# EPFL-IMOS/simple-SFOD

Hardware: AMD Instinct MI355X
Metric: teacher+student train images/s on 1024x2048 synthetic (higher is better)
Workload: dtype bf16x3

## Files before the change

### include/sfod_hip.h

```cpp
#ifndef SFOD_HIP_H
#define SFOD_HIP_H
#include <stdint.h>
#ifdef __cplusplus
extern "C" {
#endif

#define SFOD_F32 0
#define SFOD_BF16 1
#define SFOD_BF16X3 2
#define SFOD_F16X3 3

int sfod_version(void);
const char* sfod_last_error(void);

int sfod_preprocess(const void* const* img_ptrs, const int32_t* sizes, int B, int Hp, int Wp,
                    int Cpad, const float* mean3, const float* std3, void* out, int dt,
                    void* stream);

int sfod_hflip_u8(const void* src, void* dst, int C, int H, int W, void* stream);

int sfod_resize_bilinear_u8(const void* src, void* dst, int C, int H, int W, int h, int w,
                            const int32_t* hbounds, const int32_t* hcoef, int ksize_h,
                            const int32_t* vbounds, const int32_t* vcoef, int ksize_v, int flip,
                            void* stream);

int sfod_conv_fwd(const void* x, const void* w, const float* bias, void* y, int B, int H, int W,
                  int Cin, int Cout, int ksize, int ldy, int act, float* stats, int dt, int out_dt,
                  void* stream);
int sfod_conv_fwd_ws(const void* x, const void* w, const uint32_t* w_absmax, const float* bias, void* y, int B, int H,
                     int W, int Cin, int Cout, int ksize, int ldy, int act, float* stats, int dt, int out_dt,
                     void* stream);
int64_t sfod_conv_fwd_scratch_bytes(int B, int H, int W, int Cin, int Cout, int ksize, int dt, int out_dt, int with_stats);
int sfod_conv_fwd_scratch(const void* x, const void* w, const uint32_t* w_absmax, const float* bias, void* y, int B, int H,
                          int W, int Cin, int Cout, int ksize, int ldy, int act, float* stats, int dt, int out_dt,
                          void* scratch, int64_t scratch_bytes, void* stream);
int sfod_conv_stats_blocks(int B, int H, int W, int Cin, int Cout, int ksize, int dt);
int sfod_set_conv_algo(int algo);
int sfod_conv_dgrad_bnred_blocks(int B, int H, int W, int Cin, int Cout, int dt);
int sfod_conv_dgrad_bnred(const void* x, const void* w, void* dz, int B, int H, int W, int Cin, int Cout, int dt,
                          const float* y, const float* mean, const float* invstd, const float* gamma,
                          const float* beta, float* red_ws, void* stream);
int sfod_conv_fwd_bnin_supported(int B, int H, int W, int Cin, int Cout, int dt);
int sfod_conv_fwd_bnin(const float* x_pre, const float* in_mean, const float* in_invstd, const float* in_gamma,
                       const float* in_beta, const void* w, const float* bias, float* y, int B, int H, int W, int Cin,
                       int Cout, int ldy, int act, float* stats, int dt, void* stream);
int sfod_set_gemm_tile(int tile);
int sfod_set_conv3x3_variant(int variant);
int sfod_last_conv_kernel(char* buf, int n);
int sfod_set_deterministic(int on);
int sfod_get_deterministic(void);
int sfod_set_conv3x3_m16(int on);
int sfod_set_wgrad3x3_pipe(int on);
int sfod_conv_fwd_algo(int B, int H, int W, int Cin, int Cout, int ksize, int dt);

int sfod_conv_first_supported(int B, int H, int W, int Cin, int Cout, int dt, int ldy);
int sfod_conv_first_fused(const void* x, const void* w, const float* bias, const float* scale,
                          const float* shift, void* y, float* stats, int B, int H, int W, int ldy,
                          int act, int dt, void* stream);
int sfod_conv_first_fused_ws(const void* x, const void* w, const uint32_t* w_absmax, const float* bias,
                             const float* scale, const float* shift, void* y, float* stats, int B, int H, int W,
                             int ldy, int act, int dt, void* stream);

int64_t sfod_conv_wgrad_ws_bytes(int B, int H, int W, int Cin, int Cout, int ksize, int lddy, int dt);
int sfod_conv_wgrad(const void* x, const void* dy, float* dw, int B, int H, int W, int Cin,
                    int Cout, int ksize, int lddy, int dt, void* ws, int64_t ws_bytes, void* stream);
int sfod_conv_wgrad_oihw_supported(int B, int H, int W, int Cin, int Cout, int ksize, int lddy, int dt);
int sfod_conv_wgrad_oihw(const void* x, const void* dy, float* dw_oihw, int B, int H, int W, int Cin,
                         int Cout, int ksize, int lddy, int dt, int accumulate, void* ws,
// ... 173 lines not shown
```

### simple-sfod_amd/csrc/conv3x3_patch.hip

```cpp
#include "conv_internal.h"
#include <type_traits>
#include <stdlib.h>
#include <atomic>

typedef __attribute__((ext_vector_type(8))) __bf16 bf16x8;
typedef __attribute__((ext_vector_type(16))) float f32x16;
typedef __attribute__((ext_vector_type(4))) float f32x4_t;

#define LDS_PTR(p) ((__attribute__((address_space(3))) void*)(p))

namespace {

template <int J> using IC = std::integral_constant<int, J>;

constexpr int BSLOT = 8192;
constexpr int STG_PITCH = 144;

template <int G, int FM> struct Lay {
  static constexpr bool SMALL = (G == 1) ? (FM == 2) : (FM == 1);
  static constexpr int NPW = SMALL ? 3 : 5;
  static constexpr int PATCH_ROWS = NPW * 8 * 16;
  static constexpr int PATCH_BYTES = PATCH_ROWS * 64;
  static constexpr int D = SMALL ? 2 : 3;
  static constexpr int NBS = D + 1;
// ... 11 lines not shown
  const bf16_t* x;
  const bf16_t* w;
  const float* bias;
  void* y;
  float* stats;
  int B, H, W, Cin, Cout, ldy, act;
  int TH, TW, PW;
  int tiles_x, tiles_y, tiles_n;
  unsigned m_pw, m_tw, m_tn, m_tx, m_ty;
  int nbody;
  int ntiles;
  int nblk;
  const float* red_y;
  const float* red_mean;
  const float* red_invstd;
  const float* red_gamma;
  const float* red_beta;
  float* red_ws;
  const unsigned* wamax;
  const float* xf_mean;
  const float* xf_invstd;
  const float* xf_gamma;
  const float* xf_beta;
};

constexpr unsigned OOB_OFF = 0x80000000u;
__device__ __forceinline__ void bufload16(__amdgpu_buffer_rsrc_t rsrc, unsigned voff, unsigned soff, void* l) {
  __builtin_amdgcn_raw_ptr_buffer_load_lds(rsrc, LDS_PTR(l), 16, (int)voff, (int)soff, 0, 0);
}

__device__ __forceinline__ unsigned fdiv(unsigned x, unsigned d, unsigned m) { return d == 1 ? x : __umulhi(x, m); }

template <int N> __device__ __forceinline__ void wait_vm() {
  asm volatile("s_waitcnt vmcnt(%0) lgkmcnt(0)" ::"n"(N) : "memory");
}

struct ActP { float slope; bool relu; };
__device__ __forceinline__ ActP act_params(int act) { return ActP{act == 2 ? 0.2f : 1.f, act == 1}; }
__device__ __forceinline__ float act_f(float v, ActP p) { return fmaxf(v, p.relu ? 0.f : v * p.slope); }

template <int G, int FM> struct WaitTab;
template <> struct WaitTab<1, 4> {
  static constexpr int N[9] = {2, 3, 4, 4, 4, 4, 3, 2, 2};
  static constexpr int NL[9] = {2, 2, 2, 2, 2, 2, 2, 1, 0};
};
template <> struct WaitTab<2, 2> {
  static constexpr int N[9] = {1, 4, 5, 4, 1, 2, 4, 5, 4};
  static constexpr int NL[9] = {1, 4, 5, 4, 1, 2, 2, 1, 0};
};
template <> struct WaitTab<1, 2> {
  static constexpr int N[9] = {1, 2, 2, 2, 1, 1, 1, 1, 1};
  static constexpr int NL[9] = {1, 1, 1, 1, 1, 1, 1, 1, 0};
};
template <> struct WaitTab<2, 1> {
  static constexpr int N[9] = {1, 2, 2, 2, 1, 1, 2, 2, 2};
  static constexpr int NL[9] = {1, 2, 2, 2, 1, 1, 1, 1, 0};
};

template <int G, int FM, typename OutT, int SPLIT = 0, bool RED = false>
__global__ void __launch_bounds__(512, (Lay<G, FM>::SMALL ? 4 : 2))
k_conv3x3_patch(P3Args a) {
  using L = Lay<G, FM>;
  constexpr int BN = 128 / G;
  constexpr int FN = 2;
  constexpr int WROWS = FM * 32;
  constexpr int NPW = L::NPW, PATCH_BYTES = L::PATCH_BYTES, BRING_OFF = L::BRING_OFF, D = L::D, NBS = L::NBS;
  constexpr int PIXTAB_OFF = L::PIXTAB_OFF, SRED_OFF = L::SRED_OFF;
  extern __shared__ __attribute__((aligned(16))) unsigned char smem[];

  const int lane = threadIdx.x & 63;
  const int wave = __builtin_amdgcn_readfirstlane(threadIdx.x >> 6);
  const int wm = (G == 1) ? (wave >> 1) : wave;
  const int wn = (G == 1) ? (wave & 1) : 0;
  const int h = lane >> 5;

  int bid = blockIdx.x;
  {
    const int q = a.ntiles / 8, r = a.ntiles % 8, xcd = bid % 8;
    bid = (xcd < r ? xcd * (q + 1) : r * (q + 1) + (xcd - r) * q) + bid / 8;
  }
  int t = (int)fdiv((unsigned)bid, (unsigned)a.tiles_n, a.m_tn);
  const int tn = bid - t * a.tiles_n;
  int t2 = (int)fdiv((unsigned)t, (unsigned)a.tiles_x, a.m_tx);
  const int txi = t - t2 * a.tiles_x;
// ... 262 lines not shown
      }
    const bool vec_ok = (a.ldy % 8) == 0;
    bf16_t* yo = reinterpret_cast<bf16_t*>(a.y);
#pragma unroll 4
    for (int it = 0; it < WROWS / 8; ++it) {
      const int row = it * 8 + (lane >> 3), ch = lane & 7;
      const int pix = pixtab[wm * WROWS + row];
      const int n = n0 + wn * 64 + ch * 8;
      if (pix < 0 || n >= a.Cout) continue;
      const unsigned char* src = stg + row * STG_PITCH + ch * 16;
      bf16_t* dst = yo + (ybase + pix) * a.ldy + n;
      if (vec_ok && n + 8 <= a.Cout) {
        *reinterpret_cast<uint4*>(dst) = *reinterpret_cast<const uint4*>(src);
      } else {
        for (int e = 0; e < 8 && n + e < a.Cout; ++e) dst[e] = reinterpret_cast<const bf16_t*>(src)[e];
      }
    }
  } else {
    float* yo = reinterpret_cast<float*>(a.y);
    constexpr int FP = 272;
    static_assert(8 * 32 * FP <= Lay<G, FM>::STG || 8 * 32 * FP <= Lay<G, FM>::OPER, "fp32 staging must fit the operand area");
    unsigned char* stg = smem + wave * (32 * FP);
    const bool vec_ok = (a.ldy % 4) == 0;
#pragma unroll
    for (int i = 0; i < FM; ++i) {
#pragma unroll
      for (int j = 0; j < FN; ++j) {
        const int nl = j * 32 + (lane & 31);
#pragma unroll
        for (int r = 0; r < 16; ++r) {
          const int ml = (r & 3) + 8 * (r >> 2) + 4 * h;
          const float v = acc[i][j][r] + bcol[j];
          acc[i][j][r] = v;
          *reinterpret_cast<float*>(stg + ml * FP + nl * 4) = act_f(v, actp);
        }
      }
#pragma unroll
      for (int it = 0; it < 8; ++it) {
        const int row = it * 4 + (lane >> 4), ch = lane & 15;
        const int pix = pixtab[wm * WROWS + i * 32 + row];
        const int n = n0 + wn * 64 + ch * 4;
        if (pix < 0 || n >= a.Cout) continue;
        const float4 v = *reinterpret_cast<const float4*>(stg + row * FP + ch * 16);
        float* dst = yo + (ybase + pix) * a.ldy + n;
        if (vec_ok && n + 4 <= a.Cout) {
          *reinterpret_cast<float4*>(dst) = v;
        } else {
          const float e[4] = {v.x, v.y, v.z, v.w};
          for (int q = 0; q < 4 && n + q < a.Cout; ++q) dst[q] = e[q];
        }
      }
    }
  }

  if constexpr (RED) {
    static_assert(sizeof(OutT) == 4, "the reduction epilogue belongs to fp32 data-gradient launches");
    float* sred = reinterpret_cast<float*>(smem + SRED_OFF);
    const float* __restrict__ yb = a.red_y + ybase * a.ldy;
#pragma unroll
    for (int j = 0; j < FN; ++j) {
      const int n = n0 + wn * 64 + j * 32 + (lane & 31);
      const int nc = min(n, a.Cout - 1);
      const float mu = a.red_mean[nc], is = a.red_invstd[nc];
      const float sc = is * a.red_gamma[nc], sh = a.red_beta[nc];
      float sb = 0.f, sg = 0.f;
#pragma unroll
      for (int i = 0; i < FM; ++i)
#pragma unroll
        for (int r = 0; r < 16; ++r) {
          const int ml = i * 32 + (r & 3) + 8 * (r >> 2) + 4 * h;
          const int pix = pixtab[wm * WROWS + ml];
          const float yv = yb[(unsigned)(max(pix, 0) * a.ldy + nc)];
          const float d = yv - mu;
          const float g = (pix >= 0 && d * sc + sh > 0.f) ? acc[i][j][r] : 0.f;
// ... 136 lines not shown
  }
}

template <int NW, int NIP, int NWN = 2> struct M16Lay {
  static constexpr int PIX = (NW / NWN) * NIP * 16;
  static constexpr int PR = (PIX == 256) ? 384 : 640;
  static constexpr int NPW = PR / 16 / NW;
  static constexpr int PPS = (NPW + 2) / 3;
  static constexpr int PPP = 4 * NWN;
  static constexpr int WPW = 2 * PPP / NW;
  static constexpr int PATCH_BYTES = PR * 64;
  static constexpr int WR_OFF = 2 * PATCH_BYTES;
  static constexpr int WSLOT = 2 * PPP * 1024;
  static constexpr int LDS = WR_OFF + 2 * WSLOT;
  static_assert(WPW >= 1 && PPP % WPW == 0 && PPS <= 3, "a wave's weight pieces of a stage lie inside one pair");
};

#ifdef M16_STAMP
__device__ unsigned long long g_m16_stamps[8];
#endif

typedef float __attribute__((address_space(4))) cfloat_k;

template <int NW, int NIP, int FMT, bool RED, bool XF = false, int NWN = 2>
__global__ void __launch_bounds__(NW * 64, (NW * (160 * 1024 / M16Lay<NW, NIP, NWN>::LDS)) / 4 > 0 ? (NW * (160 * 1024 / M16Lay<NW, NIP, NWN>::LDS)) / 4 : 1)
k_conv3x3_m16(P3Args a) {
  using L = M16Lay<NW, NIP, NWN>;
  static_assert(!XF || NWN == 2, "the in-LDS BatchNorm transform lives in the 128-channel shape");
  static_assert(!XF || (NW == 4 && NIP == 8 && FMT == 1 && !RED), "the in-LDS BatchNorm transform lives in the 4-wave bf16-pair forward kernel");
#ifdef M16_STAMP
  const unsigned long long stamp_t0 = __builtin_amdgcn_s_memtime();
#endif
  constexpr int PR = L::PR, NPW = L::NPW, WPW = L::WPW, PATCH_BYTES = L::PATCH_BYTES, WR_OFF = L::WR_OFF, WSLOT = L::WSLOT;
  constexpr int NWM = NW / NWN;
  constexpr int PPP = L::PPP;
  constexpr int WPX = NIP * 16;
  constexpr int XB = (NIP >= 8) ? 2 : 1;
  extern __shared__ __attribute__((aligned(16))) unsigned char smem[];

  const int lane = threadIdx.x & 63;
  const int wave = __builtin_amdgcn_readfirstlane(threadIdx.x >> 6);
  const int wm = wave / NWN, wn = wave % NWN;
  const int q = lane >> 4, r16 = lane & 15;
  const int pb = q & 1, chh = q >> 1;

  int bid = blockIdx.x;
  {
    const int qq = a.ntiles / 8, r = a.ntiles % 8, xcd = bid % 8;
    bid = (xcd < r ? xcd * (qq + 1) : r * (qq + 1) + (xcd - r) * qq) + bid / 8;
  }
// ... 312 lines not shown
    }
    pix[ip] = v;
  }
  const int cb = n0 + wn * 64 + q * 4;
  float* yo = reinterpret_cast<float*>(a.y);
  const bool fast = (a.ldy % 4) == 0 && (n0 + wn * 64 + 64 <= a.Cout);
  float bv[4][4];
#pragma unroll
  for (int ic = 0; ic < 4; ++ic)
#pragma unroll
    for (int r = 0; r < 4; ++r) {
      const int c = cb + ic * 16 + r;
      bv[ic][r] = (a.bias != nullptr && c < a.Cout) ? a.bias[c] : 0.f;
    }
  int64_t rowoff[NIP];
#pragma unroll
  for (int ip = 0; ip < NIP; ++ip) rowoff[ip] = (ybase + max(pix[ip], 0)) * a.ldy;
#pragma unroll
  for (int ic = 0; ic < 4; ++ic)
#pragma unroll
    for (int ip = 0; ip < NIP; ++ip)
#pragma unroll
      for (int r = 0; r < 4; ++r) acc[ic][ip][r] += bv[ic][r];
  if (fast) {
#pragma unroll
    for (int ic = 0; ic < 4; ++ic)
#pragma unroll
      for (int ip = 0; ip < NIP; ++ip) {
        float4 o;
        o.x = act_f(acc[ic][ip][0], actp); o.y = act_f(acc[ic][ip][1], actp);
        o.z = act_f(acc[ic][ip][2], actp); o.w = act_f(acc[ic][ip][3], actp);
        if (pix[ip] >= 0) *reinterpret_cast<float4*>(yo + rowoff[ip] + (cb + ic * 16)) = o;
      }
  } else {
#pragma unroll
    for (int ic = 0; ic < 4; ++ic)
#pragma unroll
      for (int ip = 0; ip < NIP; ++ip)
#pragma unroll
        for (int r = 0; r < 4; ++r) {
          const int c = cb + ic * 16 + r;
          if (pix[ip] >= 0 && c < a.Cout) yo[rowoff[ip] + c] = act_f(acc[ic][ip][r], actp);
        }
  }

  if constexpr (!RED) { if (a.stats == nullptr) return; }
  __syncthreads();
// ... 194 lines not shown
  p.G = (variant <= 2) ? 1 : 2;
  p.FM = (variant == 1) ? 4 : (variant == 3 ? 1 : 2);
  if (Cin % (32 * p.G) != 0) return p;
  if ((int64_t)H * W * Cin >= (int64_t)1 << 30 || (int64_t)Cout * 9 * Cin >= (int64_t)1 << 30) return p;
  const int BM = (p.G == 1 ? 4 : 8) * p.FM * 32;
  const int cap = (BM == 256) ? PATCH_ROWS_SMALL : PATCH_ROWS_BIG;
  if (!p3_best_tile(H, W, BM, cap, p.TH, p.TW, p.tiles_y, p.tiles_x)) return p;
  p.tiles_n = (Cout + (128 / p.G) - 1) / (128 / p.G);
  p.nblk = B * p.tiles_y * p.tiles_x;
  p.ok = 1;
  return p;
}

#ifdef M16_STAMP
extern "C" int sfod_debug_m16_stamps(unsigned long long* out8, int reset) {
  SFOD_REQUIRE_EXTENTS("debug_m16_stamps", reset);
  hipDeviceSynchronize();
  hipMemcpyFromSymbol(out8, HIP_SYMBOL(g_m16_stamps), 64);
  if (reset) { unsigned long long z[8] = {0, 0, 0, 0, 0, 0, 0, 0}; hipMemcpyToSymbol(HIP_SYMBOL(g_m16_stamps), z, 64); }
  return 0;
}
#endif

template <int NW, int NIP, int FMT, bool RED, bool XF = false, int NWN = 2>
static int p3_launch_m16(P3Args a, hipStream_t s) {
  auto kern = k_conv3x3_m16<NW, NIP, FMT, RED, XF, NWN>;
  constexpr int LDS = M16Lay<NW, NIP, NWN>::LDS;
  static const hipError_t attr_rc =
      hipFuncSetAttribute(reinterpret_cast<const void*>(kern), hipFuncAttributeMaxDynamicSharedMemorySize, LDS);
  if (attr_rc != hipSuccess) { sfod_set_error("hipFuncSetAttribute(m16): %s", hipGetErrorString(attr_rc)); return -(int)attr_rc; }
  a.nbody = a.Cin / 64;
  static const std::string kname =
      sfod_kernel_name("k_conv3x3_m16<%d,%d,%d,%d,%d,%d>", NW, NIP, FMT, (int)RED, (int)XF, NWN);
  sfod_note_conv_kernel(kname.c_str());
  hipLaunchKernelGGL(kern, dim3(a.ntiles), dim3(NW * 64), LDS, s, a);
  return sfod_check_launch("conv3x3_m16");
}

template <int G, int FM, typename OutT, int SPLIT = 0, bool RED = false>
static int p3_launch_one(const P3Args& a, hipStream_t s) {
  auto kern = k_conv3x3_patch<G, FM, OutT, SPLIT, RED>;
  constexpr int LDS = Lay<G, FM>::TOTAL;
  static const hipError_t attr_rc =
      hipFuncSetAttribute(reinterpret_cast<const void*>(kern), hipFuncAttributeMaxDynamicSharedMemorySize, LDS);
  if (attr_rc != hipSuccess) { sfod_set_error("hipFuncSetAttribute(p3): %s", hipGetErrorString(attr_rc)); return -(int)attr_rc; }
  static const std::string kname =
      sfod_kernel_name("k_conv3x3_patch<%d,%d,%s,%d,%d>", G, FM, sfod_type_name<OutT>(), SPLIT, (int)RED);
  sfod_note_conv_kernel(kname.c_str());
  hipLaunchKernelGGL(kern, dim3(a.ntiles), dim3(512), LDS, s, a);
  return sfod_check_launch("conv3x3_patch");
}

bool sfod_p3_bnin_ok(const P3Plan& p, int Cin_phys, int split) {
  return p.ok && p.m16 != 0 && p.G == 1 && p.FM == 2 && Cin_phys % 64 == 0 && split == 1;
}

int sfod_p3_launch(const P3Plan& p, const void* x, const void* w, const float* bias, void* y, float* stats,
                   int B, int H, int W, int Cin, int Cout, int ldy, int act, int out_f32, hipStream_t s, int split,
                   const P3BnRed* red, const unsigned* wamax, const P3BnIn* bnin) {
  P3Args a;
  a.wamax = wamax;
  a.xf_mean = a.xf_invstd = a.xf_gamma = a.xf_beta = nullptr;
  if (bnin != nullptr) {
    if (!sfod_p3_bnin_ok(p, Cin, split) || red != nullptr || !out_f32) {
      sfod_set_error("conv3x3_patch: the BatchNorm-input form needs bf16x3 operands, the 256 x 128 shape, Cin % 32 == 0");
      return SFOD_EBADARG;
    }
    a.xf_mean = bnin->mean; a.xf_invstd = bnin->invstd; a.xf_gamma = bnin->gamma; a.xf_beta = bnin->beta;
  }
  a.red_y = nullptr; a.red_mean = a.red_invstd = a.red_gamma = a.red_beta = nullptr; a.red_ws = nullptr;
  if (red != nullptr) {
    if (!out_f32 || ldy != Cout || Cout % 4 != 0) { sfod_set_error("conv3x3_patch: BatchNorm-backward epilogue needs a dense fp32 output"); return SFOD_EBADARG; }
    a.red_y = red->y; a.red_mean = red->mean; a.red_invstd = red->invstd; a.red_gamma = red->gamma; a.red_beta = red->beta;
    a.red_ws = red->ws;
  }
  a.x = (const bf16_t*)x; a.w = (const bf16_t*)w; a.bias = bias; a.y = y; a.stats = stats;
  a.B = B; a.H = H; a.W = W; a.Cin = Cin; a.Cout = Cout; a.ldy = ldy; a.act = act;
  a.TH = p.TH; a.TW = p.TW; a.PW = p.TW + 2;
  a.tiles_x = p.tiles_x; a.tiles_y = p.tiles_y; a.tiles_n = p.tiles_n;
  auto magic = [](int d) { return (unsigned)((((unsigned long long)1) << 32) / (unsigned)d + 1ull); };
  a.m_pw = magic(a.PW); a.m_tw = magic(a.TW); a.m_tn = magic(a.tiles_n); a.m_tx = magic(a.tiles_x);
  a.m_ty = magic(a.tiles_y);
  a.nbody = Cin / (32 * p.G);
  a.ntiles = B * p.tiles_y * p.tiles_x * p.tiles_n;
  a.nblk = p.nblk;
  if (split) {
    if (!out_f32) { sfod_set_error("conv3x3_patch: operand pairs write fp32"); return SFOD_EBADARG; }
    if (bnin != nullptr) return p3_launch_m16<4, 8, 1, false, true>(a, s);
    if (p.m16 && p.G == 1 && p.FM == 2 && Cin % 64 == 0 && (red == nullptr || split == 1)) {
      if (p.m16 == 2) {
        if (red != nullptr) return p3_launch_m16<4, 8, 1, true>(a, s);
        return split == 2 ? p3_launch_m16<4, 8, 2, false>(a, s) : p3_launch_m16<4, 8, 1, false>(a, s);
      }
      if (red != nullptr) return p3_launch_m16<8, 4, 1, true>(a, s);
      return split == 2 ? p3_launch_m16<8, 4, 2, false>(a, s) : p3_launch_m16<8, 4, 1, false>(a, s);
    }
    if (p.m16 && p.G == 2 && Cin % 64 == 0 && (red == nullptr || split == 1) && (p.m16 >= 3 || p3_m16_n64_enabled())) {
      if (p.FM == 1 && (p.m16 == 4 || p3_m16_n64_enabled() == 2)) {
        if (red != nullptr) return p3_launch_m16<8, 2, 1, true, false, 1>(a, s);
        return split == 2 ? p3_launch_m16<8, 2, 2, false, false, 1>(a, s) : p3_launch_m16<8, 2, 1, false, false, 1>(a, s);
      }
      if (p.FM == 1) {
        if (red != nullptr) return p3_launch_m16<4, 4, 1, true, false, 1>(a, s);
        return split == 2 ? p3_launch_m16<4, 4, 2, false, false, 1>(a, s) : p3_launch_m16<4, 4, 1, false, false, 1>(a, s);
      }
      if (red != nullptr) return p3_launch_m16<8, 4, 1, true, false, 1>(a, s);
      return split == 2 ? p3_launch_m16<8, 4, 2, false, false, 1>(a, s) : p3_launch_m16<8, 4, 1, false, false, 1>(a, s);
    }
    if (red != nullptr) {
      if (split != 1) { sfod_set_error("conv3x3_patch: the BatchNorm-backward epilogue runs on bf16x3 operands"); return SFOD_EBADARG; }
      if (p.G == 1 && p.FM == 2) return p3_launch_one<1, 2, float, 1, true>(a, s);
// ... 21 lines not shown
```

### simple-sfod_amd/csrc/conv_internal.h

```cpp
#pragma once
#include "common.h"

struct P3Plan {
  int ok;
  int G;
  int FM;
  int TH, TW;
  int tiles_y, tiles_x, tiles_n;
  int nblk;
  int m16;
};
P3Plan sfod_p3_plan(int B, int H, int W, int Cin, int Cout, int pairs = 0);
struct P3BnRed {
  const float* y;
  const float* mean;
  const float* invstd;
  const float* gamma;
  const float* beta;
  float* ws;
};
struct P3BnIn {
  const float* mean;
  const float* invstd;
  const float* gamma;
  const float* beta;
};
bool sfod_p3_bnin_ok(const P3Plan& p, int Cin_phys, int split);
int sfod_p3_launch(const P3Plan& p, const void* x, const void* w, const float* bias, void* y, float* stats,
                   int B, int H, int W, int Cin, int Cout, int ldy, int act, int out_f32, hipStream_t s, int split = 0,
                   const P3BnRed* red = nullptr, const unsigned* wamax = nullptr, const P3BnIn* bnin = nullptr);


struct W3Plan {
  int ok;
  int CO;
  int TH, TW, tiles_y, tiles_x;
  int co_tiles, ci_tiles;
  int tiles_per_split, nsplit, nslab;
  int64_t ws_bytes;
  int w64;
};
W3Plan sfod_w3_plan(int B, int H, int W, int Cin, int Cout, int lddy, int split = 0);
int sfod_w3_launch(const W3Plan& p, const void* x, const void* dy, float* dw, void* ws, int B, int H, int W,
                   int Cin, int Cout, int lddy, int out_mode, hipStream_t s, int split = 0);

bool sfod_deterministic();

void sfod_f16_poll_elementwise(unsigned* out, hipStream_t s);
void sfod_f16_poll_roi(unsigned* out, hipStream_t s);
void sfod_f16_poll_first(unsigned* out, hipStream_t s);
void sfod_f16_poll_stem(unsigned* out, hipStream_t s);

int sfod_f1_nblk(int B, int H, int W);
// ... 4 lines not shown
```

### simple-sfod_amd/csrc/gemm_conv.hip

```cpp
#include "conv_internal.h"
#include <algorithm>
#include <atomic>

typedef __attribute__((ext_vector_type(8))) __bf16 bf16x8;
typedef __attribute__((ext_vector_type(4))) short s16x4;
typedef __attribute__((ext_vector_type(8))) short s16x8;
typedef __attribute__((ext_vector_type(16))) float f32x16;
typedef __attribute__((ext_vector_type(4))) float f32x4;

#define LDS_PTR(p) ((__attribute__((address_space(3))) void*)(p))
#define GLB_PTR(p) ((const __attribute__((address_space(1))) void*)(p))

__device__ __attribute__((aligned(16))) unsigned int g_zero_page[64];

struct ConvArgs {
  int M;
  int H, W;
  int Cin;
  int Cout;
  int ks;
  int cpt_shift;
  int kchunks;
  int ldy;
  int act;
// ... 732 lines not shown
extern "C" int sfod_conv_fwd_bnin_supported(int B, int H, int W, int Cin, int Cout, int dt) {
  if (!conv_shape_fits(B, H, W, Cin, Cout, 3)) return 0;
  if (dt != SFOD_BF16X3 || (int64_t)B * H * W == 0 || g_conv_algo == 1) return 0;
  const int pc = phys_ch(dt, Cin);
  const P3Plan p = sfod_p3_plan(B, H, W, pc, Cout, 1);
  return (use_patch_kernel(p, B, H, W, 3, dt) && sfod_p3_bnin_ok(p, pc, 1)) ? 1 : 0;
}

extern "C" int sfod_conv_fwd_bnin(const float* x_pre, const float* in_mean, const float* in_invstd, const float* in_gamma,
                                  const float* in_beta, const void* w, const float* bias, float* y, int B, int H, int W,
                                  int Cin, int Cout, int ldy, int act, float* stats, int dt, void* stream) {
  sfod_note_conv_kernel(nullptr);
  SFOD_REQUIRE(conv_shape_fits(B, H, W, Cin, Cout, 3) && sfod_ints_ok({ldy}), "conv_fwd_bnin: negative or oversized extent");
  SFOD_REQUIRE(sfod_conv_fwd_bnin_supported(B, H, W, Cin, Cout, dt), "conv_fwd_bnin: shape not served (sfod_conv_fwd_bnin_supported)");
  SFOD_REQUIRE(x_pre && in_mean && in_invstd && in_gamma && in_beta && w && y, "conv_fwd_bnin: null argument");
  SFOD_REQUIRE(ldy >= Cout, "conv_fwd_bnin: ldy < Cout");
  const int pc = phys_ch(dt, Cin);
  const P3Plan p = sfod_p3_plan(B, H, W, pc, Cout, 1);
  const P3BnIn bnin{in_mean, in_invstd, in_gamma, in_beta};
  return sfod_p3_launch(p, x_pre, w, bias, y, stats, B, H, W, pc, Cout, ldy, act, 1, (hipStream_t)stream, 1, nullptr, nullptr,
                        &bnin);
}

extern "C" int sfod_conv_dgrad_bnred_blocks(int B, int H, int W, int Cin, int Cout, int dt) {
  if (!conv_shape_fits(B, H, W, Cin, Cout, 3)) return 0;
  if (dt != SFOD_BF16X3 && dt != SFOD_BF16) return 0;
  if (dt == SFOD_BF16) return 0;
  if (Cout % 4 != 0) return 0;
  const P3Plan p = sfod_p3_plan(B, H, W, phys_ch(dt, Cin), Cout, sfod_is_pairs(dt));
  return use_patch_kernel(p, B, H, W, 3, dt) ? p.nblk : 0;
}

extern "C" int sfod_conv_dgrad_bnred(const void* x, const void* w, void* dz, int B, int H, int W, int Cin, int Cout,
                                     int dt, const float* y, const float* mean, const float* invstd,
                                     const float* gamma, const float* beta, float* red_ws, void* stream) {
  sfod_note_conv_kernel(nullptr);
  SFOD_REQUIRE(conv_shape_fits(B, H, W, Cin, Cout, 3), "conv_dgrad_bnred: negative or oversized extent");
  SFOD_REQUIRE(x != nullptr && w != nullptr && dz != nullptr, "conv_dgrad_bnred: null operand");
  SFOD_REQUIRE(sfod_conv_dgrad_bnred_blocks(B, H, W, Cin, Cout, dt) > 0,
               "conv_dgrad_bnred: shape not served (sfod_conv_dgrad_bnred_blocks)");
  SFOD_REQUIRE(y && mean && invstd && gamma && beta && red_ws, "conv_dgrad_bnred: null argument");
  const int pc = phys_ch(dt, Cin);
  const P3Plan p = sfod_p3_plan(B, H, W, pc, Cout, sfod_is_pairs(dt));
  const P3BnRed red{y, mean, invstd, gamma, beta, red_ws};
  return sfod_p3_launch(p, x, w, nullptr, dz, nullptr, B, H, W, pc, Cout, Cout, 0, 1, (hipStream_t)stream,
                        dt == SFOD_BF16X3, &red);
// ... 648 lines not shown
```

### simple-sfod_amd/modeling/backbone_vgg.py

```python
import os

import torch
import torch.nn as nn

from .. import native
from . import offchain as _offchain
from ..registry import BACKBONE_REGISTRY
from ..structures import ShapeSpec

VGG16 = [64, 64, "M", 128, 128, "M", 256, 256, 256, "M", 512, 512, 512, "M", 512, 512, 512, "M"]
STAGE_SLICES = [(0, 7), (7, 14), (14, 24), (24, 34), (34, 44)]


def make_layers(cfg_list, batch_norm=False):
    layers = []
    in_channels = 3
    for v in cfg_list:
        if v == "M":
            layers += [nn.MaxPool2d(kernel_size=2, stride=2)]
        else:
            conv2d = nn.Conv2d(in_channels, v, kernel_size=3, padding=1)
            if batch_norm:
                layers += [conv2d, nn.BatchNorm2d(v), nn.ReLU(inplace=True)]
            else:
# ... 44 lines not shown
        self._initialize_weights()
        chans, strides = [64, 128, 256, 512, 512], [2, 4, 8, 16, 32]
        mods = list(self.vgg._modules.values())
        self.stages = [nn.Sequential(*mods[a:b]) for a, b in STAGE_SLICES]
        self._out_feature_channels, self._out_feature_strides, self._stage_names = {}, {}, []
        for i, stage in enumerate(self.stages):
            name = "vgg{}".format(i)
            self.add_module(name, stage)
            self._stage_names.append(name)
            self._out_feature_channels[name] = chans[i]
            self._out_feature_strides[name] = strides[i]
        self._out_features = self._stage_names
        self.needed_features = set(self._stage_names)
        del self.vgg
        self.compute_dtype = native.mode_dtype(cfg.SFOD.COMPUTE_DTYPE)
        self.grad_dtype = native.grad_dtype_of(self.compute_dtype)
        self.bn_momentum, self.bn_eps = 0.1, 1e-5
        self.bn_updates_per_forward = 1
        self.fuse_first = bool(cfg.SFOD.FUSE_FIRST_LAYER) if "SFOD" in cfg and "FUSE_FIRST_LAYER" in cfg.SFOD else True
        self.fuse_bn_input = bool(cfg.SFOD.FUSE_BN_INPUT) if "SFOD" in cfg and "FUSE_BN_INPUT" in cfg.SFOD else True
        self.fuse_bn_input_min_bytes = int(os.environ.get("SFOD_BNIN_MIN_BYTES", str(256 << 20)))
        self.wgrad_stream = os.environ.get("SFOD_VGG_WGRAD_STREAM", "1") != "0"
        self.fuse_bn_reduce = os.environ.get("SFOD_NO_FUSE_BN_REDUCE", "0") != "1"
        self._plan = []
        for s, stage in enumerate(self.stages):
            ms = list(stage)
            i = 0
            while i < len(ms):
                if isinstance(ms[i], nn.Conv2d):
                    pool = i + 3 < len(ms) and isinstance(ms[i + 3], nn.MaxPool2d)
                    self._plan.append([ms[i], ms[i + 1], pool, False])
                    i += 4 if pool else 3
                else:
                    i += 1
            self._plan[-1][3] = True

    @property
    def size_divisibility(self):
        return 0

    def output_shape(self):
        return {n: ShapeSpec(channels=self._out_feature_channels[n], stride=self._out_feature_strides[n])
                for n in self._out_features}

    def _initialize_weights(self):
        for m in self.modules():
# ... 58 lines not shown
            fwd = [(conv.weight, cin0_pad if li == 0 else conv.in_channels, False)
                   for li, (conv, _, _, _) in enumerate(self._plan)]
            rot = [(conv.weight, conv.out_channels, True) for conv, _, _, _ in self._plan[1:]] if with_dgrad else []
            if gdt == dt or not rot:
                pk = (native.ConvWeightPacker(fwd + rot, dt), None)
            else:
                pk = (native.ConvWeightPacker(fwd, dt), native.ConvWeightPacker(rot, gdt))
            packers[key] = pk
        views = list(pk[0].pack()) + (list(pk[1].pack()) if pk[1] is not None else [])
        n = len(self._plan)
        return views[:n], ([None] + list(views[n:]) if with_dgrad else None)

    def _defer_bn(self, li, y, fwd_w, save, training):
        if save or not training or not self.fuse_bn_input or li + 1 >= len(self._plan):
            return False
        _, _, pool, stage_end = self._plan[li]
        if pool or stage_end:
            return False
        if y.numel() * 4 < self.fuse_bn_input_min_bytes:
            return False
        nxt = self._plan[li + 1][0]
        return native.conv_fwd_bnin_supported(y, fwd_w[li + 1], nxt.out_channels)

    def _forward_impl(self, x, save=True):
        dt = native.dt_of(x)
        training = self.training
        saved, outs = [], []
        fwd_w, rot_w = self._packed_weights(dt, x.shape[-1], save)
        self._rot_w = rot_w
        x_g = native.as_operand(x, self.grad_dtype) if save else None
        pending = None
        for li, (conv, bn, pool, stage_end) in enumerate(self._plan):
            cout = conv.out_channels
            wp = fwd_w[li]
            if pending is not None:
                yb, mb, ib, bnb = pending
                pending = None
                B, H, W, _ = yb.shape
                y, stats = native.conv_fwd_bnin(yb, mb, ib, bnb.weight.detach(), bnb.bias.detach(), wp, conv.bias.detach(),
                                                cout, want_stats=True)
                mean, invstd = native.bn_finalize(stats, B * H * W, cout, bn.running_mean, bn.running_var,
                                                  self.bn_momentum, self.bn_eps, self.bn_updates_per_forward,
                                                  num_batches_tracked=bn.num_batches_tracked)
                if self._defer_bn(li, y, fwd_w, save, training):
                    pending = (y, mean, invstd, bn)
                    continue
                x = native.bn_relu_pool_fwd(y, mean, invstd, bn.weight.detach(), bn.bias.detach(), pool, out_dtype=x.dtype)
                if stage_end:
                    outs.append(x)
                continue
            B, H, W, _ = x.shape
            if (li == 0 and training and not save and not pool and not stage_end and self.fuse_first
                    and native.conv_first_supported(x, cout)):
                stats = native.conv_first_stats(x, wp, conv.bias.detach())
                mean, invstd = native.bn_finalize(stats, B * H * W, cout, bn.running_mean, bn.running_var,
                                                  self.bn_momentum, self.bn_eps, self.bn_updates_per_forward,
                                                  num_batches_tracked=bn.num_batches_tracked)
                scale = bn.weight.detach() * invstd
                shift = bn.bias.detach() - mean * scale
                x = native.conv_first_apply(x, wp, conv.bias.detach(), scale, shift, relu=True)
                continue
            if training:
                y, stats = native.conv_fwd(x, wp, conv.bias.detach(), cout, 3, want_stats=True)
                mean, invstd = native.bn_finalize(stats, B * H * W, cout, bn.running_mean, bn.running_var,
                                                  self.bn_momentum, self.bn_eps, self.bn_updates_per_forward,
                                                  num_batches_tracked=bn.num_batches_tracked)
            else:
                y = native.conv_fwd(x, wp, conv.bias.detach(), cout, 3)
                mean = bn.running_mean
                invstd = torch.rsqrt(bn.running_var + self.bn_eps)
            if self._defer_bn(li, y, fwd_w, save, training):
                pending = (y, mean, invstd, bn)
                continue
            zz = native.bn_relu_pool_fwd(y, mean, invstd, bn.weight.detach(), bn.bias.detach(), pool,
# ... 96 lines not shown
```

### simple-sfod_amd/native.py

```python
import ctypes
import os
import re
import warnings

import torch

warnings.filterwarnings("ignore", message="ComplexHalf support is experimental")

_HERE = os.path.dirname(os.path.abspath(__file__))
HEADER = os.path.join(os.path.dirname(_HERE), "include", "sfod_hip.h")
SO_PATH = os.environ.get("SFOD_HIP_LIB", os.path.join(_HERE, "lib", "libsfod_hip.so"))

F32, BF16, BF16X3, F16X3 = 0, 1, 2, 3

SPLIT_DTYPE = torch.complex32
SPLITH_DTYPE = torch.uint32
PAIR_DTYPES = (SPLIT_DTYPE, SPLITH_DTYPE)

COMPUTE_MODES = {"fp32": F32, "bf16": BF16, "bf16x3": BF16X3, "f16x3": F16X3}


def mode_dt(name):
    try:
        return COMPUTE_MODES[str(name).lower()]
# ... 538 lines not shown
    _pending_flops = 2.0 * B * H * W * cout * ksize * ksize * cin
    if _timer is not None:
        _pending_tag = ":patch3x3" if query("sfod_conv_fwd_algo", B, H, W, cin, cout, ksize, dt) == 2 else ":gemm"
    odt = dt_of_dtype(out_dtype)
    nscratch = load().sfod_conv_fwd_scratch_bytes(B, H, W, cin, cout, ksize, dt, odt, int(want_stats)) if ksize == 1 else 0
    if nscratch > 0:
        scratch = torch.empty(nscratch, dtype=torch.uint8, device=x.device)
        call("sfod_conv_fwd_scratch", x, w_packed, wscale_of(w_packed), bias, y, B, H, W, cin, cout, ksize, ldy, act, stats,
             dt, odt, scratch, nscratch, timer_name="sfod_conv_fwd")
    else:
        call("sfod_conv_fwd_ws", x, w_packed, wscale_of(w_packed), bias, y, B, H, W, cin, cout, ksize, ldy, act, stats, dt,
             odt, timer_name="sfod_conv_fwd")
    _pending_tag = ""
    return (y, stats) if want_stats else y


def conv_fwd_bnin_supported(y_pre, w_packed, cout):
    if y_pre.dim() != 4 or y_pre.dtype != torch.float32 or w_packed.dtype != SPLIT_DTYPE:
        return False
    B, H, W, cin = y_pre.shape
    return bool(query("sfod_conv_fwd_bnin_supported", B, H, W, cin, cout, BF16X3))


def conv_fwd_bnin(y_pre, mean, invstd, gamma, beta, w_packed, bias, cout, act=0, want_stats=False):
    B, H, W, cin = y_pre.shape
    y = torch.empty((B, H, W, cout), dtype=torch.float32, device=y_pre.device)
    stats = None
    if want_stats:
        nb = query("sfod_conv_stats_blocks", B, H, W, cin, cout, 3, BF16X3)
        stats = torch.empty(nb * (2 * cout + 1), dtype=torch.float32, device=y_pre.device)
        stats.nblk = nb
    global _pending_flops, _pending_tag
    _pending_flops = 2.0 * B * H * W * cout * 9 * cin
    _pending_tag = ":patch3x3"
    try:
        call("sfod_conv_fwd_bnin", y_pre, mean, invstd, gamma, beta, w_packed, bias, y, B, H, W, cin, cout, cout, act, stats,
             BF16X3, timer_name="sfod_conv_fwd")
    finally:
        _pending_tag = ""
    return (y, stats) if want_stats else y


def conv_first_supported(x, cout):
    if x.dim() != 4 or x.dtype not in (torch.bfloat16,) + PAIR_DTYPES:
        return False
    B, H, W, cin = x.shape
    return bool(query("sfod_conv_first_supported", B, H, W, cin, cout, dt_of(x), cout))


def conv_first_stats(x, w_packed, bias):
    B, H, W, cin = x.shape
    nb = query("sfod_conv_stats_blocks", B, H, W, cin, 64, 3, dt_of(x))
    stats = torch.empty(nb * (2 * 64 + 1), dtype=torch.float32, device=x.device)
    stats.nblk = nb
    call("sfod_conv_first_fused_ws", x, w_packed, wscale_of(w_packed), bias, None, None, None, stats, B, H, W, 64, 0,
         dt_of(x))
    return stats


def conv_first_apply(x, w_packed, bias, scale, shift, relu=True):
    B, H, W, cin = x.shape
    z = torch.empty(B, H, W, 64, dtype=x.dtype, device=x.device)
    global _pending_flops
# ... 536 lines not shown
```

Before: 160.4.

## Fuse 2x2 max-pool into conv3x3 forward epilogue for teacher forward

Adds a pooling epilogue to the patch and m16 3x3 conv kernels. Each 2x2 window is reduced with a sign-aware max, using the BN gamma sign so the max commutes with the later affine BN, and only the pooled map is written. The backbone uses it when no activations are saved (the teacher forward), so the full-resolution fp32 conv output is never written or reread by the pool pass. The cost is extra epilogue work, LDS staging or DPP shuffles, and new template instantiations. Correctness depends on the sign trick and on BN statistics still being gathered at full resolution.

Measured after the change: 161.6, median of 6. About the same (+0.8%).

```diff
diff --git a/include/sfod_hip.h b/include/sfod_hip.h
--- a/include/sfod_hip.h
+++ b/include/sfod_hip.h
@@ -44,6 +44,12 @@
 int sfod_conv_fwd_bnin(const float* x_pre, const float* in_mean, const float* in_invstd, const float* in_gamma,
                        const float* in_beta, const void* w, const float* bias, float* y, int B, int H, int W, int Cin,
                        int Cout, int ldy, int act, float* stats, int dt, void* stream);
+int sfod_conv_fwd_pool_supported(int B, int H, int W, int Cin, int Cout, int dt, int bnin);
+int sfod_conv_fwd_pool(const void* x, const void* w, const float* bias, const float* pool_gamma, float* y_pooled, int B,
+                       int H, int W, int Cin, int Cout, int ldy, float* stats, int dt, void* stream);
+int sfod_conv_fwd_bnin_pool(const float* x_pre, const float* in_mean, const float* in_invstd, const float* in_gamma,
+                            const float* in_beta, const void* w, const float* bias, const float* pool_gamma, float* y_pooled,
+                            int B, int H, int W, int Cin, int Cout, int ldy, float* stats, int dt, void* stream);
 int sfod_set_gemm_tile(int tile);
 int sfod_set_conv3x3_variant(int variant);
 int sfod_last_conv_kernel(char* buf, int n);
diff --git a/simple-sfod_amd/csrc/conv3x3_patch.hip b/simple-sfod_amd/csrc/conv3x3_patch.hip
--- a/simple-sfod_amd/csrc/conv3x3_patch.hip
+++ b/simple-sfod_amd/csrc/conv3x3_patch.hip
@@ -57,7 +57,15 @@
   const float* xf_invstd;
   const float* xf_gamma;
   const float* xf_beta;
+  const float* pool_gamma;
 };
+
+__device__ __forceinline__ unsigned pool_sign(const float* g, int n, int Cout) {
+  return (n < Cout) ? (__builtin_bit_cast(unsigned, g[n]) & 0x80000000u) : 0u;
+}
+__device__ __forceinline__ float pool_flip(float v, unsigned sg) {
+  return __builtin_bit_cast(float, __builtin_bit_cast(unsigned, v) ^ sg);
+}
 
 constexpr unsigned OOB_OFF = 0x80000000u;
 __device__ __forceinline__ void bufload16(__amdgpu_buffer_rsrc_t rsrc, unsigned voff, unsigned soff, void* l) {
@@ -92,9 +100,10 @@
   static constexpr int NL[9] = {1, 2, 2, 2, 1, 1, 1, 1, 0};
 };
 
-template <int G, int FM, typename OutT, int SPLIT = 0, bool RED = false>
+template <int G, int FM, typename OutT, int SPLIT = 0, bool RED = false, bool POOL = false>
 __global__ void __launch_bounds__(512, (Lay<G, FM>::SMALL ? 4 : 2))
 k_conv3x3_patch(P3Args a) {
+  static_assert(!POOL || (G == 2 && FM == 1 && sizeof(OutT) == 4 && !RED), "the pooling epilogue lives in the 256 x 64 fp32 forward shape");
   using L = Lay<G, FM>;
   constexpr int BN = 128 / G;
   constexpr int FN = 2;
@@ -403,6 +412,49 @@
     static_assert(8 * 32 * FP <= Lay<G, FM>::STG || 8 * 32 * FP <= Lay<G, FM>::OPER, "fp32 staging must fit the operand area");
     unsigned char* stg = smem + wave * (32 * FP);
     const bool vec_ok = (a.ldy % 4) == 0;
+    if constexpr (POOL) {
+#pragma unroll
+      for (int j = 0; j < FN; ++j) {
+        const int nl = j * 32 + (lane & 31);
+#pragma unroll
+        for (int r = 0; r < 16; ++r) {
+          const int ml = (r & 3) + 8 * (r >> 2) + 4 * h;
+          const float v = acc[0][j][r] + bcol[j];
+          acc[0][j][r] = v;
+          *reinterpret_cast<float*>(stg + ml * FP + nl * 4) = v;
+        }
+      }
+      __syncthreads();
+      const int pw2 = a.TW >> 1, np2 = (a.TH >> 1) * pw2;
+      const int Hp = a.H >> 1, Wp = a.W >> 1;
+      for (int it = threadIdx.x; it < np2 * 16; it += 512) {
+        const int pp = it >> 4, ch = it & 15;
+        const int pr = pp / pw2, pc = pp - pr * pw2;
+        const int ty = 2 * pr, tx = 2 * pc;
+        const int n = n0 + ch * 4;
+        if (y0 + ty + 1 >= a.H || x0 + tx + 1 >= a.W || n >= a.Cout) continue;
+        const unsigned char* src = smem + (ty * a.TW + tx) * FP + ch * 16;
+        const float4 v00 = *reinterpret_cast<const float4*>(src), v01 = *reinterpret_cast<const float4*>(src + FP);
+        const float4 v10 = *reinterpret_cast<const float4*>(src + a.TW * FP);
+        const float4 v11 = *reinterpret_cast<const float4*>(src + (a.TW + 1) * FP);
+        const float e00[4] = {v00.x, v00.y, v00.z, v00.w}, e01[4] = {v01.x, v01.y, v01.z, v01.w};
+        const float e10[4] = {v10.x, v10.y, v10.z, v10.w}, e11[4] = {v11.x, v11.y, v11.z, v11.w};
+        float o[4];
+#pragma unroll
+        for (int q = 0; q < 4; ++q) {
+          const unsigned sg = pool_sign(a.pool_gamma, n + q, a.Cout);
+          const float m = fmaxf(fmaxf(pool_flip(e00[q], sg), pool_flip(e01[q], sg)),
+                                fmaxf(pool_flip(e10[q], sg), pool_flip(e11[q], sg)));
+          o[q] = pool_flip(m, sg);
+        }
+        float* dst = yo + (((int64_t)b * Hp + ((y0 + ty) >> 1)) * Wp + ((x0 + tx) >> 1)) * a.ldy + n;
+        if (vec_ok && n + 4 <= a.Cout) {
+          *reinterpret_cast<float4*>(dst) = make_float4(o[0], o[1], o[2], o[3]);
+        } else {
+          for (int q = 0; q < 4 && n + q < a.Cout; ++q) dst[q] = o[q];
+        }
+      }
+    } else {
 #pragma unroll
     for (int i = 0; i < FM; ++i) {
 #pragma unroll
@@ -431,6 +483,7 @@
           for (int q = 0; q < 4 && n + q < a.Cout; ++q) dst[q] = e[q];
         }
       }
+    }
     }
   }
 
@@ -613,10 +666,11 @@
 
 typedef float __attribute__((address_space(4))) cfloat_k;
 
-template <int NW, int NIP, int FMT, bool RED, bool XF = false, int NWN = 2>
+template <int NW, int NIP, int FMT, bool RED, bool XF = false, int NWN = 2, bool POOL = false>
 __global__ void __launch_bounds__(NW * 64, (NW * (160 * 1024 / M16Lay<NW, NIP, NWN>::LDS)) / 4 > 0 ? (NW * (160 * 1024 / M16Lay<NW, NIP, NWN>::LDS)) / 4 : 1)
 k_conv3x3_m16(P3Args a) {
   using L = M16Lay<NW, NIP, NWN>;
+  static_assert(!POOL || (NW == 4 && NIP == 8 && NWN == 2 && !RED), "the pooling epilogue lives in the 4-wave 256 x 128 forward shape");
   static_assert(!XF || NWN == 2, "the in-LDS BatchNorm transform lives in the 128-channel shape");
   static_assert(!XF || (NW == 4 && NIP == 8 && FMT == 1 && !RED), "the in-LDS BatchNorm transform lives in the 4-wave bf16-pair forward kernel");
 #ifdef M16_STAMP
@@ -975,7 +1029,41 @@
     for (int ip = 0; ip < NIP; ++ip)
 #pragma unroll
       for (int r = 0; r < 4; ++r) acc[ic][ip][r] += bv[ic][r];
-  if (fast) {
+  if constexpr (POOL) {
+    const int Hp = a.H >> 1, Wp = a.W >> 1;
+    unsigned sg[4][4];
+#pragma unroll
+    for (int ic = 0; ic < 4; ++ic)
+#pragma unroll
+      for (int r = 0; r < 4; ++r) sg[ic][r] = pool_sign(a.pool_gamma, cb + ic * 16 + r, a.Cout);
+#pragma unroll
+    for (int ipp = 0; ipp < NIP / 2; ++ipp) {
+      const int ip = (ipp >> 1) * 4 + (ipp & 1);
+      const int p = wm * WPX + ip * 16 + r16;
+      const int ty = p >> 5, tx = p & 31;
+      const bool ok = (r16 & 1) == 0 && ty + 1 < a.TH && y0 + ty + 1 < a.H && x0 + tx + 1 < a.W;
+      const int64_t off = (((int64_t)b * Hp + ((y0 + ty) >> 1)) * Wp + ((x0 + tx) >> 1)) * a.ldy;
+#pragma unroll
+      for (int ic = 0; ic < 4; ++ic) {
+        float o[4];
+#pragma unroll
+        for (int r = 0; r < 4; ++r) {
+          float m = fmaxf(pool_flip(acc[ic][ip][r], sg[ic][r]), pool_flip(acc[ic][ip + 2][r], sg[ic][r]));
+          m = fmaxf(m, __builtin_bit_cast(float, __builtin_amdgcn_update_dpp(0, __builtin_bit_cast(int, m), 0xB1, 0xF, 0xF, true)));
+          o[r] = pool_flip(m, sg[ic][r]);
+        }
+        if (ok) {
+          if (fast) {
+            *reinterpret_cast<float4*>(yo + off + (cb + ic * 16)) = make_float4(o[0], o[1], o[2], o[3]);
+          } else {
+#pragma unroll
+            for (int r = 0; r < 4; ++r)
+              if (cb + ic * 16 + r < a.Cout) yo[off + cb + ic * 16 + r] = o[r];
+          }
+        }
+      }
+    }
+  } else if (fast) {
 #pragma unroll
     for (int ic = 0; ic < 4; ++ic)
 #pragma unroll
@@ -1216,30 +1304,32 @@
 }
 #endif
 
-template <int NW, int NIP, int FMT, bool RED, bool XF = false, int NWN = 2>
+template <int NW, int NIP, int FMT, bool RED, bool XF = false, int NWN = 2, bool POOL = false>
 static int p3_launch_m16(P3Args a, hipStream_t s) {
-  auto kern = k_conv3x3_m16<NW, NIP, FMT, RED, XF, NWN>;
+  auto kern = k_conv3x3_m16<NW, NIP, FMT, RED, XF, NWN, POOL>;
   constexpr int LDS = M16Lay<NW, NIP, NWN>::LDS;
   static const hipError_t attr_rc =
       hipFuncSetAttribute(reinterpret_cast<const void*>(kern), hipFuncAttributeMaxDynamicSharedMemorySize, LDS);
   if (attr_rc != hipSuccess) { sfod_set_error("hipFuncSetAttribute(m16): %s", hipGetErrorString(attr_rc)); return -(int)attr_rc; }
   a.nbody = a.Cin / 64;
-  static const std::string kname =
-      sfod_kernel_name("k_conv3x3_m16<%d,%d,%d,%d,%d,%d>", NW, NIP, FMT, (int)RED, (int)XF, NWN);
+  static const std::string kname = POOL
+      ? sfod_kernel_name("k_conv3x3_m16<%d,%d,%d,%d,%d,%d,1>", NW, NIP, FMT, (int)RED, (int)XF, NWN)
+      : sfod_kernel_name("k_conv3x3_m16<%d,%d,%d,%d,%d,%d>", NW, NIP, FMT, (int)RED, (int)XF, NWN);
   sfod_note_conv_kernel(kname.c_str());
   hipLaunchKernelGGL(kern, dim3(a.ntiles), dim3(NW * 64), LDS, s, a);
   return sfod_check_launch("conv3x3_m16");
 }
 
-template <int G, int FM, typename OutT, int SPLIT = 0, bool RED = false>
+template <int G, int FM, typename OutT, int SPLIT = 0, bool RED = false, bool POOL = false>
 static int p3_launch_one(const P3Args& a, hipStream_t s) {
-  auto kern = k_conv3x3_patch<G, FM, OutT, SPLIT, RED>;
+  auto kern = k_conv3x3_patch<G, FM, OutT, SPLIT, RED, POOL>;
   constexpr int LDS = Lay<G, FM>::TOTAL;
   static const hipError_t attr_rc =
       hipFuncSetAttribute(reinterpret_cast<const void*>(kern), hipFuncAttributeMaxDynamicSharedMemorySize, LDS);
   if (attr_rc != hipSuccess) { sfod_set_error("hipFuncSetAttribute(p3): %s", hipGetErrorString(attr_rc)); return -(int)attr_rc; }
-  static const std::string kname =
-      sfod_kernel_name("k_conv3x3_patch<%d,%d,%s,%d,%d>", G, FM, sfod_type_name<OutT>(), SPLIT, (int)RED);
+  static const std::string kname = POOL
+      ? sfod_kernel_name("k_conv3x3_patch<%d,%d,%s,%d,%d,1>", G, FM, sfod_type_name<OutT>(), SPLIT, (int)RED)
+      : sfod_kernel_name("k_conv3x3_patch<%d,%d,%s,%d,%d>", G, FM, sfod_type_name<OutT>(), SPLIT, (int)RED);
   sfod_note_conv_kernel(kname.c_str());
   hipLaunchKernelGGL(kern, dim3(a.ntiles), dim3(512), LDS, s, a);
   return sfod_check_launch("conv3x3_patch");
@@ -1249,11 +1339,25 @@
   return p.ok && p.m16 != 0 && p.G == 1 && p.FM == 2 && Cin_phys % 64 == 0 && split == 1;
 }
 
+bool sfod_p3_pool_ok(const P3Plan& p, int Cin_phys, int split, bool bnin) {
+  if (!p.ok || split != 1 || (p.TH & 1) || (p.TW & 1)) return false;
+  if (bnin) return sfod_p3_bnin_ok(p, Cin_phys, split) && p.TW == 32;
+  if (p.G != 2 || p.FM != 1 || Cin_phys % 64 != 0) return false;
+  return !(p.m16 && (p.m16 >= 3 || p3_m16_n64_enabled()));
+}
+
 int sfod_p3_launch(const P3Plan& p, const void* x, const void* w, const float* bias, void* y, float* stats,
                    int B, int H, int W, int Cin, int Cout, int ldy, int act, int out_f32, hipStream_t s, int split,
-                   const P3BnRed* red, const unsigned* wamax, const P3BnIn* bnin) {
+                   const P3BnRed* red, const unsigned* wamax, const P3BnIn* bnin, const float* pool_gamma) {
   P3Args a;
   a.wamax = wamax;
+  a.pool_gamma = pool_gamma;
+  if (pool_gamma != nullptr) {
+    if (!sfod_p3_pool_ok(p, Cin, split, bnin != nullptr) || red != nullptr || !out_f32 || act != 0 || wamax != nullptr) {
+      sfod_set_error("conv3x3_patch: the pooling epilogue needs bf16x3 operands, act none and an even tile of a shape it serves");
+      return SFOD_EBADARG;
+    }
+  }
   a.xf_mean = a.xf_invstd = a.xf_gamma = a.xf_beta = nullptr;
   if (bnin != nullptr) {
     if (!sfod_p3_bnin_ok(p, Cin, split) || red != nullptr || !out_f32) {
@@ -1280,7 +1384,9 @@
   a.nblk = p.nblk;
   if (split) {
     if (!out_f32) { sfod_set_error("conv3x3_patch: operand pairs write fp32"); return SFOD_EBADARG; }
+    if (bnin != nullptr && pool_gamma != nullptr) return p3_launch_m16<4, 8, 1, false, true, 2, true>(a, s);
     if (bnin != nullptr) return p3_launch_m16<4, 8, 1, false, true>(a, s);
+    if (pool_gamma != nullptr) return p3_launch_one<2, 1, float, 1, false, true>(a, s);
     if (p.m16 && p.G == 1 && p.FM == 2 && Cin % 64 == 0 && (red == nullptr || split == 1)) {
       if (p.m16 == 2) {
         if (red != nullptr) return p3_launch_m16<4, 8, 1, true>(a, s);
diff --git a/simple-sfod_amd/csrc/conv_internal.h b/simple-sfod_amd/csrc/conv_internal.h
--- a/simple-sfod_amd/csrc/conv_internal.h
+++ b/simple-sfod_amd/csrc/conv_internal.h
@@ -26,9 +26,11 @@
   const float* beta;
 };
 bool sfod_p3_bnin_ok(const P3Plan& p, int Cin_phys, int split);
+bool sfod_p3_pool_ok(const P3Plan& p, int Cin_phys, int split, bool bnin);
 int sfod_p3_launch(const P3Plan& p, const void* x, const void* w, const float* bias, void* y, float* stats,
                    int B, int H, int W, int Cin, int Cout, int ldy, int act, int out_f32, hipStream_t s, int split = 0,
-                   const P3BnRed* red = nullptr, const unsigned* wamax = nullptr, const P3BnIn* bnin = nullptr);
+                   const P3BnRed* red = nullptr, const unsigned* wamax = nullptr, const P3BnIn* bnin = nullptr,
+                   const float* pool_gamma = nullptr);
 
 
 struct W3Plan {
diff --git a/simple-sfod_amd/csrc/gemm_conv.hip b/simple-sfod_amd/csrc/gemm_conv.hip
--- a/simple-sfod_amd/csrc/gemm_conv.hip
+++ b/simple-sfod_amd/csrc/gemm_conv.hip
@@ -778,6 +778,45 @@
                         &bnin);
 }
 
+extern "C" int sfod_conv_fwd_pool_supported(int B, int H, int W, int Cin, int Cout, int dt, int bnin) {
+  if (!conv_shape_fits(B, H, W, Cin, Cout, 3)) return 0;
+  if (dt != SFOD_BF16X3 || (int64_t)B * H * W == 0 || g_conv_algo == 1) return 0;
+  if (bnin && !sfod_conv_fwd_bnin_supported(B, H, W, Cin, Cout, dt)) return 0;
+  if (!bnin && use_first_kernel(B, H, W, Cin, Cout, 3, dt, Cout, SFOD_F32)) return 0;
+  const int pc = phys_ch(dt, Cin);
+  const P3Plan p = sfod_p3_plan(B, H, W, pc, Cout, 1);
+  return (use_patch_kernel(p, B, H, W, 3, dt) && sfod_p3_pool_ok(p, pc, 1, bnin != 0)) ? 1 : 0;
+}
+
+extern "C" int sfod_conv_fwd_pool(const void* x, const void* w, const float* bias, const float* pool_gamma, float* y_pooled,
+                                  int B, int H, int W, int Cin, int Cout, int ldy, float* stats, int dt, void* stream) {
+  sfod_note_conv_kernel(nullptr);
+  SFOD_REQUIRE(conv_shape_fits(B, H, W, Cin, Cout, 3) && sfod_ints_ok({ldy}), "conv_fwd_pool: negative or oversized extent");
+  SFOD_REQUIRE(sfod_conv_fwd_pool_supported(B, H, W, Cin, Cout, dt, 0), "conv_fwd_pool: shape not served (sfod_conv_fwd_pool_supported)");
+  SFOD_REQUIRE(x && w && pool_gamma && y_pooled, "conv_fwd_pool: null argument");
+  SFOD_REQUIRE(ldy >= Cout, "conv_fwd_pool: ldy < Cout");
+  const int pc = phys_ch(dt, Cin);
+  const P3Plan p = sfod_p3_plan(B, H, W, pc, Cout, 1);
+  return sfod_p3_launch(p, x, w, bias, y_pooled, stats, B, H, W, pc, Cout, ldy, 0, 1, (hipStream_t)stream, 1, nullptr, nullptr,
+                        nullptr, pool_gamma);
+}
+
+extern "C" int sfod_conv_fwd_bnin_pool(const float* x_pre, const float* in_mean, const float* in_invstd, const float* in_gamma,
+                                       const float* in_beta, const void* w, const float* bias, const float* pool_gamma,
+                                       float* y_pooled, int B, int H, int W, int Cin, int Cout, int ldy, float* stats, int dt,
+                                       void* stream) {
+  sfod_note_conv_kernel(nullptr);
+  SFOD_REQUIRE(conv_shape_fits(B, H, W, Cin, Cout, 3) && sfod_ints_ok({ldy}), "conv_fwd_bnin_pool: negative or oversized extent");
+  SFOD_REQUIRE(sfod_conv_fwd_pool_supported(B, H, W, Cin, Cout, dt, 1), "conv_fwd_bnin_pool: shape not served (sfod_conv_fwd_pool_supported)");
+  SFOD_REQUIRE(x_pre && in_mean && in_invstd && in_gamma && in_beta && w && pool_gamma && y_pooled, "conv_fwd_bnin_pool: null argument");
+  SFOD_REQUIRE(ldy >= Cout, "conv_fwd_bnin_pool: ldy < Cout");
+  const int pc = phys_ch(dt, Cin);
+  const P3Plan p = sfod_p3_plan(B, H, W, pc, Cout, 1);
+  const P3BnIn bnin{in_mean, in_invstd, in_gamma, in_beta};
+  return sfod_p3_launch(p, x_pre, w, bias, y_pooled, stats, B, H, W, pc, Cout, ldy, 0, 1, (hipStream_t)stream, 1, nullptr, nullptr,
+                        &bnin, pool_gamma);
+}
+
 extern "C" int sfod_conv_dgrad_bnred_blocks(int B, int H, int W, int Cin, int Cout, int dt) {
   if (!conv_shape_fits(B, H, W, Cin, Cout, 3)) return 0;
   if (dt != SFOD_BF16X3 && dt != SFOD_BF16) return 0;
diff --git a/simple-sfod_amd/modeling/backbone_vgg.py b/simple-sfod_amd/modeling/backbone_vgg.py
--- a/simple-sfod_amd/modeling/backbone_vgg.py
+++ b/simple-sfod_amd/modeling/backbone_vgg.py
@@ -90,6 +90,7 @@
         self.fuse_bn_input_min_bytes = int(os.environ.get("SFOD_BNIN_MIN_BYTES", str(256 << 20)))
         self.wgrad_stream = os.environ.get("SFOD_VGG_WGRAD_STREAM", "1") != "0"
         self.fuse_bn_reduce = os.environ.get("SFOD_NO_FUSE_BN_REDUCE", "0") != "1"
+        self.pool_epilogue = os.environ.get("SFOD_POOL_EPILOGUE", "1") != "0"
         self._plan = []
         for s, stage in enumerate(self.stages):
             ms = list(stage)
@@ -194,6 +195,11 @@
         nxt = self._plan[li + 1][0]
         return native.conv_fwd_bnin_supported(y, fwd_w[li + 1], nxt.out_channels)
 
+    def _pool_in_epilogue(self, x, w_packed, cout, save, training, bnin=False):
+        if save or not training or not self.pool_epilogue:
+            return False
+        return native.conv_fwd_pool_supported(x, w_packed, cout, bnin=bnin)
+
     def _forward_impl(self, x, save=True):
         dt = native.dt_of(x)
         training = self.training
@@ -209,19 +215,30 @@
                 yb, mb, ib, bnb = pending
                 pending = None
                 B, H, W, _ = yb.shape
+                pooled = pool and self._pool_in_epilogue(yb, wp, cout, save, training, bnin=True)
                 y, stats = native.conv_fwd_bnin(yb, mb, ib, bnb.weight.detach(), bnb.bias.detach(), wp, conv.bias.detach(),
-                                                cout, want_stats=True)
+                                                cout, want_stats=True, pool_gamma=bn.weight.detach() if pooled else None)
                 mean, invstd = native.bn_finalize(stats, B * H * W, cout, bn.running_mean, bn.running_var,
                                                   self.bn_momentum, self.bn_eps, self.bn_updates_per_forward,
                                                   num_batches_tracked=bn.num_batches_tracked)
                 if self._defer_bn(li, y, fwd_w, save, training):
                     pending = (y, mean, invstd, bn)
                     continue
-                x = native.bn_relu_pool_fwd(y, mean, invstd, bn.weight.detach(), bn.bias.detach(), pool, out_dtype=x.dtype)
+                x = native.bn_relu_pool_fwd(y, mean, invstd, bn.weight.detach(), bn.bias.detach(), pool and not pooled,
+                                            out_dtype=x.dtype)
                 if stage_end:
                     outs.append(x)
                 continue
             B, H, W, _ = x.shape
+            if pool and self._pool_in_epilogue(x, wp, cout, save, training):
+                y, stats = native.conv_fwd_pool(x, wp, conv.bias.detach(), bn.weight.detach(), cout)
+                mean, invstd = native.bn_finalize(stats, B * H * W, cout, bn.running_mean, bn.running_var,
+                                                  self.bn_momentum, self.bn_eps, self.bn_updates_per_forward,
+                                                  num_batches_tracked=bn.num_batches_tracked)
+                x = native.bn_relu_pool_fwd(y, mean, invstd, bn.weight.detach(), bn.bias.detach(), False, out_dtype=x.dtype)
+                if stage_end:
+                    outs.append(x)
+                continue
             if (li == 0 and training and not save and not pool and not stage_end and self.fuse_first
                     and native.conv_first_supported(x, cout)):
                 stats = native.conv_first_stats(x, wp, conv.bias.detach())
diff --git a/simple-sfod_amd/native.py b/simple-sfod_amd/native.py
--- a/simple-sfod_amd/native.py
+++ b/simple-sfod_amd/native.py
@@ -584,7 +584,10 @@
     return bool(query("sfod_conv_fwd_bnin_supported", B, H, W, cin, cout, BF16X3))
 
 
-def conv_fwd_bnin(y_pre, mean, invstd, gamma, beta, w_packed, bias, cout, act=0, want_stats=False):
+def conv_fwd_bnin(y_pre, mean, invstd, gamma, beta, w_packed, bias, cout, act=0, want_stats=False, pool_gamma=None):
+    if pool_gamma is not None:
+        assert act == 0 and want_stats
+        return conv_fwd_bnin_pool(y_pre, mean, invstd, gamma, beta, w_packed, bias, pool_gamma, cout)
     B, H, W, cin = y_pre.shape
     y = torch.empty((B, H, W, cout), dtype=torch.float32, device=y_pre.device)
     stats = None
@@ -601,6 +604,50 @@
     finally:
         _pending_tag = ""
     return (y, stats) if want_stats else y
+
+
+def conv_fwd_pool_supported(x, w_packed, cout, bnin=False):
+    if x.dim() != 4 or w_packed.dtype != SPLIT_DTYPE or x.dtype != (torch.float32 if bnin else SPLIT_DTYPE):
+        return False
+    B, H, W, cin = x.shape
+    return bool(query("sfod_conv_fwd_pool_supported", B, H, W, cin, cout, BF16X3, int(bool(bnin))))
+
+
+def _pooled_out(x, cout):
+    B, H, W, cin = x.shape
+    y = torch.empty((B, H // 2, W // 2, cout), dtype=torch.float32, device=x.device)
+    nb = query("sfod_conv_stats_blocks", B, H, W, cin, cout, 3, BF16X3)
+    stats = torch.empty(nb * (2 * cout + 1), dtype=torch.float32, device=x.device)
+    stats.nblk = nb
+    return y, stats
+
+
+def conv_fwd_pool(x, w_packed, bias, pool_gamma, cout):
+    B, H, W, cin = x.shape
+    y, stats = _pooled_out(x, cout)
+    global _pending_flops, _pending_tag
+    _pending_flops = 2.0 * B * H * W * cout * 9 * cin
+    _pending_tag = ":patch3x3"
+    try:
+        call("sfod_conv_fwd_pool", x, w_packed, bias, pool_gamma, y, B, H, W, cin, cout, cout, stats, BF16X3,
+             timer_name="sfod_conv_fwd")
+    finally:
+        _pending_tag = ""
+    return y, stats
+
+
+def conv_fwd_bnin_pool(y_pre, mean, invstd, gamma, beta, w_packed, bias, pool_gamma, cout):
+    B, H, W, cin = y_pre.shape
+    y, stats = _pooled_out(y_pre, cout)
+    global _pending_flops, _pending_tag
+    _pending_flops = 2.0 * B * H * W * cout * 9 * cin
+    _pending_tag = ":patch3x3"
+    try:
+        call("sfod_conv_fwd_bnin_pool", y_pre, mean, invstd, gamma, beta, w_packed, bias, pool_gamma, y, B, H, W, cin, cout,
+             cout, stats, BF16X3, timer_name="sfod_conv_fwd")
+    finally:
+        _pending_tag = ""
+    return y, stats
 
 
 def conv_first_supported(x, cout):
```
